# tsnb66/afivo-streamer

Measured on AMD Instinct MI355X. Metric: cell-updates/s (fluid+MG V-cycle), higher is better.
Workload: dtype f64; 1 GPU; s1-64; n_cell=64, leaf_cells=134217728, boxes=585, levels=4, coarse_solve=exact separable, fused_rhs=interior, face_field=from phi in the flux, vcycle_graphs=False, parallelism=single-gpu

## Files before the change

afivo-streamer_amd/csrc/afh_species.hip:

```cpp
#include <algorithm>
#include <type_traits>
#include <utility>

#include "afh_internal.h"
#include "afh_networks.h"

namespace afh {

constexpr int MAXS = AFH_MAX_SPECIES;
constexpr int MAXPREV = 4;

__device__ __forceinline__ size_t fidx(int nf, int d, int i, int j, int k) {
  return (size_t)d * nf * nf * nf + ((size_t)(k - 1) * nf + (j - 1)) * nf +
         (i - 1);
}

struct DevLT {
  int n_points, n_cols;
  double x_min, inv_fac;
  const double *rc;
  const double *rm = nullptr;
};

__device__ __forceinline__ double lt_col(const DevLT &lt, int col, double x) {
// ... 564 lines not shown
  const double *c = R.c;
  const double Tg = A.Tg;
  const double kB = 1.3806503e-23, eV = 1.6022e-19;
  const double electron_eV_to_K = 2 * eV / (3 * kB);
  if ((R.rate_type == AFH_RATE_K1 || R.rate_type == AFH_RATE_K3) && Te < 0)
    Te = electron_eV_to_K * lt_col(A.td, A.te_col, field);
  switch (R.rate_type) {
  case AFH_RATE_K1: return c0 * c[0] * pow(300 / Te, c[1]);
  case AFH_RATE_K3: {
    const double z = (kB / eV) * Te + c[1];
    return c0 * (c[0] * (z * z) - c[2]) * c[3];
  }
  case AFH_RATE_K4: return c0 * c[0] * pow(Tg / 300, c[1]) * exp(-c[2] / Tg);
  case AFH_RATE_K5: return c0 * c[0] * exp(-c[1] / Tg);
  case AFH_RATE_K6: return c0 * c[0] * pow(Tg, c[1]);
  case AFH_RATE_K7: return c0 * c[0] * pow(Tg / c[1], c[2]);
  case AFH_RATE_K8: return c0 * c[0] * pow(300 / Tg, c[1]);
  case AFH_RATE_K9: return c0 * c[0] * exp(-c[1] * Tg);
  case AFH_RATE_K10: return c0 * pow(10.0, c[0] + c[1] * (Tg - 300));
  case AFH_RATE_K11: return c0 * c[0] * pow(300 / Tg, c[1]) * exp(-c[2] / Tg);
  case AFH_RATE_K12: return c0 * c[0] * pow(Tg, c[1]) * exp(-c[2] / Tg);
  case AFH_RATE_K13: return c0 * c[0] * exp(-pow(c[1] / (c[2] + field), c[3]));
  case AFH_RATE_K14: return c0 * c[0] * exp(-pow(field / c[1], c[2]));
  default:
    return c0 * c[0] * exp(-pow(c[1] / (kB * (Tg + field / c[2])), c[3]));
  }
}

__device__ __forceinline__ double lt_at_rm(const DevLT &lt, int col, int low, double lf) {
  const double *r = lt.rm + (size_t)(low - 1) * lt.n_cols + (col - 1);
  return lf * r[0] + (1 - lf) * r[lt.n_cols];
}

template <bool SLOW>
__device__ __forceinline__ double rate_of(const UpdArgs &A, const DevReaction &R,
                                          double field, double &Te, int low = -1,
                                          double lf = 0.0) {
  const double c0 = R.rate_factor;
  const double *c = R.c;
  switch (R.rate_type) {
  case AFH_RATE_TABULATED_FIELD:
    return c0 * (low > 0 ? lt_at_rm(A.chem, R.table_col, low, lf)
                         : lt_col(A.chem, R.table_col, field));
  case AFH_RATE_CONSTANT: return c0 * c[0];
  case AFH_RATE_LINEAR: return c0 * c[0] * (field - c[1]);
  case AFH_RATE_EXP_V1: {
    const double z = c[1] / (c[2] + field);
    return c0 * c[0] * exp(-(z * z));
  }
  case AFH_RATE_EXP_V2: {
    const double z = field / c[1];
    return c0 * c[0] * exp(-(z * z));
  }
  default: return SLOW ? rate_slow(A, R, field, Te) : 0.0;
  }
}

template <int T, bool SLOW>
__device__ __forceinline__ double rate_t(const UpdArgs &A, const DevReaction &R, double field,
                                         double &Te, int low, double lf) {
  const double c0 = R.rate_factor;
  const double *c = R.c;
  if constexpr (T == AFH_RATE_TABULATED_FIELD) {
    return c0 * (low > 0 ? lt_at_rm(A.chem, R.table_col, low, lf)
                         : lt_col(A.chem, R.table_col, field));
  } else if constexpr (T == AFH_RATE_CONSTANT) {
    return c0 * c[0];
  } else if constexpr (T == AFH_RATE_LINEAR) {
    return c0 * c[0] * (field - c[1]);
  } else if constexpr (T == AFH_RATE_EXP_V1) {
    const double z = c[1] / (c[2] + field);
    return c0 * c[0] * exp(-(z * z));
  } else if constexpr (T == AFH_RATE_EXP_V2) {
    const double z = field / c[1];
    return c0 * c[0] * exp(-(z * z));
  } else {
    static_assert(SLOW, "temperature-dependent rate form in a fast update");
    return rate_slow(A, R, field, Te);
  }
}

template <class NET>
constexpr bool net_slow() {
  for (int r = 0; r < NET::NR; r++)
    if (NET::type[r] > AFH_RATE_EXP_V2) return true;
  return false;
}

template <class NET>
constexpr int net_slot(int ix) {
  return ix <= NET::NG ? NET::NS + ix - 1 : ix - NET::NG - 1;
}

template <class NET, bool SLOW, int R, int NT>
__device__ __forceinline__ void net_one(const UpdArgs &A, double field, double &Te, int clow,
                                        double clf, const double (&dens)[NT], double (&der)[NT]) {
  constexpr int NI = NET::n_in[R], NO = NET::n_out[R];
  const DevReaction &X = A.reac[R];
  double rate = rate_t<NET::type[R], SLOW>(A, X, field, Te, clow, clf);
  double prod = 1.0;
  if constexpr (NI > 0) prod = prod * dens[net_slot<NET>(NET::ix_in[R][0])];
  if constexpr (NI > 1) prod = prod * dens[net_slot<NET>(NET::ix_in[R][1])];
  if constexpr (NI > 2) prod = prod * dens[net_slot<NET>(NET::ix_in[R][2])];
  if constexpr (NI > 3) prod = prod * dens[net_slot<NET>(NET::ix_in[R][3])];
  rate = rate * prod;
  if constexpr (NI > 0) der[net_slot<NET>(NET::ix_in[R][0])] += -rate;
  if constexpr (NI > 1) der[net_slot<NET>(NET::ix_in[R][1])] += -rate;
  if constexpr (NI > 2) der[net_slot<NET>(NET::ix_in[R][2])] += -rate;
  if constexpr (NI > 3) der[net_slot<NET>(NET::ix_in[R][3])] += -rate;
  if constexpr (NO > 0) der[net_slot<NET>(NET::ix_out[R][0])] += rate * NET::mult[R][0];
  if constexpr (NO > 1) der[net_slot<NET>(NET::ix_out[R][1])] += rate * NET::mult[R][1];
  if constexpr (NO > 2) der[net_slot<NET>(NET::ix_out[R][2])] += rate * NET::mult[R][2];
  if constexpr (NO > 3) der[net_slot<NET>(NET::ix_out[R][3])] += rate * NET::mult[R][3];
}

template <class NET, bool SLOW, int NT, size_t... R>
__device__ __forceinline__ void net_all(const UpdArgs &A, double field, double &Te, int clow,
                                        double clf, const double (&dens)[NT], double (&der)[NT],
                                        std::index_sequence<R...>) {
  (net_one<NET, SLOW, (int)R, NT>(A, field, Te, clow, clf, dens, der), ...);
}

template <class NET>
struct net_nr {
  static constexpr int v = NET::NR;
};
template <>
struct net_nr<void> {
  static constexpr int v = 1;
};

template <class NET>
static bool net_matches(const afh_fluid_desc *d) {
  const bool gas = d->i_gas_dens > 0;
  if (d->n_species != NET::NS || d->n_reactions != NET::NR || gas != (NET::GAS != 0) ||
      (gas && d->n_gas_species != NET::NG))
    return false;
  for (int r = 0; r < NET::NR; r++) {
    const afh_reaction &a = d->reactions[r];
    if (a.rate_type != NET::type[r] || a.n_in != NET::n_in[r] || a.n_out != NET::n_out[r])
      return false;
    for (int q = 0; q < a.n_in; q++)
      if (a.ix_in[q] != NET::ix_in[r][q]) return false;
    for (int q = 0; q < a.n_out; q++)
      if (a.ix_out[q] != NET::ix_out[r][q] || a.mult_out[q] != NET::mult[r][q]) return false;
  }
  return true;
}

#ifndef AFH_FLUX_LDS_NT
// ... 538 lines not shown
#undef AFH_NET_CASE
  default: break;
  }
  if (A.Ng)
    hipLaunchKernelGGL((k_update<NS, true, MAXPREV, true, true>), grid, dim3(256), 0,
                       t->stream, A, ids, nc, t->bsz, t->fsz, red);
  else if (slow && A.n_prev == 1 && !sd)
    hipLaunchKernelGGL((k_update<NS, true, 1, false>), grid, dim3(256), 0, t->stream, A,
                       ids, nc, t->bsz, t->fsz, red);
  else if (slow && A.n_prev == 2 && !sd)
    hipLaunchKernelGGL((k_update<NS, true, 2, false>), grid, dim3(256), 0, t->stream, A,
                       ids, nc, t->bsz, t->fsz, red);
  else if (slow)
    hipLaunchKernelGGL((k_update<NS, true>), grid, dim3(256), 0, t->stream, A,
                       ids, nc, t->bsz, t->fsz, red);
  else if (A.n_prev == 1 && !sd)
    hipLaunchKernelGGL((k_update<NS, false, 1, false>), grid, dim3(256), 0,
                       t->stream, A, ids, nc, t->bsz, t->fsz, red);
  else if (A.n_prev == 2 && !sd)
    hipLaunchKernelGGL((k_update<NS, false, 2, false>), grid, dim3(256), 0,
                       t->stream, A, ids, nc, t->bsz, t->fsz, red);
  else
    hipLaunchKernelGGL((k_update<NS, false>), grid, dim3(256), 0, t->stream, A,
                       ids, nc, t->bsz, t->fsz, red);
}

#ifndef AFH_FE_NT
#define AFH_FE_NT 256
#endif
#ifndef AFH_FE_MINW
#define AFH_FE_MINW 3
#endif
constexpr int FE_CHEM_LDS = 2048;
template <int NC, int LIM, int NS, int NP, bool SD, bool PHI = false, class NET = void,
          bool WF = false, int NTT = AFH_FE_NT>
__global__ void __launch_bounds__(NTT, AFH_FE_MINW)
    k_fe_lds(FluxArgs A, UpdArgs U, const double *__restrict__ tdi,
             const int32_t *__restrict__ ids, size_t bsz, size_t fsz,
             unsigned long long *red) {
  constexpr bool wf = WF;
  using G = FluxLds<NC, NTT>;
  constexpr int NG = NC + 2, NF = NC + 1, TJ = G::TJ, NT = G::NT, RW = G::RW,
                NR = G::NR, EW = G::EW, ER = G::ER, NPE = G::NPE, EPE = G::EPE;
  constexpr int SK = NG * NG, FSK = NF * NF, FD = NF * NF * NF;
  constexpr int NN = NC * NC;
  constexpr bool HAS_NET = !std::is_void<NET>::value;
  extern __shared__ double T[];
  __shared__ double SN[2][NR * RW], SE[2][ER * EW];
  __shared__ double sv[NT], sd[NT], sf[NT];
  __shared__ double r1[NT / 64], r2[NT / 64], r3[NT / 64], r4[NT / 64];
  const int tid = threadIdx.x;
  const int wg = xcd_swizzle(blockIdx.x, gridDim.x);
  const int id = ids[wg / G::NTILE];
  const int i = tid % NC + 1;
  const int jr = tid / NC;
  const int j0 = (wg % G::NTILE) * TJ + 1, j = j0 + jr;
  const size_t boff = (size_t)(id - 1) * bsz;
  const double *ne = A.ne + boff;
  const double *E = A.E + boff;
  const double *Ef = A.Ef + (size_t)(id - 1) * fsz;
  const double *ph = PHI ? A.phi + boff : nullptr;
  double *F = A.F + (size_t)(id - 1) * fsz;
  const double *g2 = A.gc2 + (size_t)(id - 1) * 6 * NN;
  const double ix = A.inv_dx[0], iy = A.inv_dx[1], iz = A.inv_dx[2];
  const double gfx = A.gfac[0], gfy = A.gfac[1], gfz = A.gfac[2];
  const double N_inv = A.N_inv;
  const int np = A.td.n_points;
  const int eix = U.e_index, dq = U.der_q, ns = HAS_NET ? NS : U.ns;
  for (int e = tid; e < 2 * np; e += NT) T[e] = tdi[e];
  constexpr int NRS = net_nr<NET>::v;
  __shared__ DevReaction sreac[NRS];
  if (HAS_NET) {
    const int nw = (int)(sizeof(DevReaction) / sizeof(int)) * NRS;
    for (int e = tid; e < nw; e += NT)
      reinterpret_cast<int *>(sreac)[e] = reinterpret_cast<const int *>(U.reac)[e];
  }
  UpdArgs Ul = U;
  if (HAS_NET) Ul.reac = sreac;
  if constexpr (HAS_NET) {
    double *Tc = T + 2 * np;
    const int nch = U.chem.n_points * U.chem.n_cols;
    for (int e = tid; e < nch; e += NT) Tc[e] = U.chem.rm[e];
    Ul.chem.rm = Tc;
  }

  auto ne_at = [&](int k, int e) -> double {
    if (e >= NR * RW) return 0.0;
    const int jj = j0 - 2 + e / RW, ii = e % RW - 1;
    const bool jin = jj >= 0 && jj <= NC + 1, iin = ii >= 0 && ii <= NC + 1;
    if (jin && iin) return ne[(k * NG + jj) * NG + ii];
    if (jin && jj >= 1 && jj <= NC) {
      if (ii == -1) return g2[0 * NN + (k - 1) * NC + (jj - 1)];
      if (ii == NC + 2) return g2[1 * NN + (k - 1) * NC + (jj - 1)];
    }
    if (iin && ii >= 1 && ii <= NC) {
      if (jj == -1) return g2[2 * NN + (k - 1) * NC + (ii - 1)];
      if (jj == NC + 2) return g2[3 * NN + (k - 1) * NC + (ii - 1)];
    }
    return 0.0;
  };
  auto e_at = [&](int k, int e) -> double {
    if (e >= ER * EW) return 0.0;
    return E[(k * NG + (j0 - 1 + e / EW)) * NG + e % EW];
  };
  const int cc = j * NG + i;
  const int fcol = (j - 1) * NF + (i - 1);
  const int gz = (j - 1) * NC + (i - 1);
  double zm1 = ne[cc], z0 = ne[SK + cc], zp1 = ne[2 * SK + cc];
  const double zm2 = g2[4 * NN + gz];
#pragma unroll
  for (int q = 0; q < NPE; q++) {
    const int e = tid + NT * q;
    if (e < NR * RW) SN[1][e] = ne_at(1, e);
  }
#pragma unroll
  for (int q = 0; q < EPE; q++) {
    const int e = tid + NT * q;
    if (e < ER * EW) SE[1][e] = e_at(1, e);
  }
  double exl, eyl, exh, eyh, pk = 0.0;
  if (PHI) {
    const int c1 = SK + cc;
    pk = ph[c1];
    exl = gfx * (pk - ph[c1 - 1]);
    eyl = gfy * (pk - ph[c1 - NG]);
    exh = i == NC ? gfx * (ph[c1 + 1] - pk) : 0.0;
    eyh = (jr == TJ - 1) ? gfy * (ph[c1 + NG] - pk) : 0.0;
  } else {
    exl = Ef[fcol], eyl = Ef[FD + fcol];
    exh = i == NC ? Ef[fcol + 1] : 0.0;
    eyh = (jr == TJ - 1) ? Ef[FD + fcol + NF] : 0.0;
  }
  double mu, dcv;
  double cmax = -HUGE_VAL, smax = -HUGE_VAL, cmin = 1e100, rmax = 0.0;
  double vz_lo, dz_lo, fz_lo;
  {
    const double ezl = PHI ? gfz * (pk - ph[cc]) : Ef[2 * FD + fcol];
    const double u = upwind_t<LIM>(A.lim, zm2, zm1, z0, zp1, ezl);
    lds_mu_dc(tdi, A.td, 0.5 * (E[cc] + E[SK + cc]) * 1e21 * N_inv, mu, dcv);
    mu = mu * N_inv;
    dz_lo = dcv * N_inv;
    vz_lo = -mu * ezl;
    fz_lo = vz_lo * u - dz_lo * iz * (z0 - zm1);
    if (wf) F[2 * FD + fcol] = fz_lo;
    smax = fmax(smax, mu * u);
  }
  __syncthreads();

  const int cn = (jr + 2) * RW + (i + 1);
  const int ce = (jr + 1) * EW + i;

  for (int k = 1; k <= NC; k++) {
    const double *N0 = SN[k & 1], *E0p = SE[k & 1];
    const bool more = k < NC;
    const double zp2 = k + 2 <= NC + 1 ? ne[(k + 2) * SK + cc]
                                       : g2[5 * NN + gz];
    const double ep1 = E[(k + 1) * SK + cc];
    const int fbn = k * FSK + fcol;
    const int x = k * SK + cc;
    double ezh, nexl = 0, neyl = 0, nexh = 0, neyh = 0, npk = 0;
    if (PHI) {
      const int cn1 = (k + 1) * SK + cc;
      npk = ph[cn1];
      if (more) {
        nexl = ph[cn1 - 1];
        neyl = ph[cn1 - NG];
        if (i == NC) nexh = ph[cn1 + 1];
        if (jr == TJ - 1) neyh = ph[cn1 + NG];
      }
      ezh = gfz * (npk - pk);
    } else {
      ezh = Ef[2 * FD + fbn];
      if (more) {
        nexl = Ef[fbn];
        neyl = Ef[FD + fbn];
        if (i == NC) nexh = Ef[fbn + 1];
        if (jr == TJ - 1) neyh = Ef[FD + fbn + NF];
      }
    }
    double pv[NS][NP], dv[NS];
#pragma unroll
    for (int s = 0; s < NS; s++) {
#pragma unroll
      for (int q = 0; q < NP; q++)
        pv[s][q] = (s >= ns || (!SD && s == eix && q == dq)) ? 0.0
                                                              : (U.prev[s][q] + boff)[x];
      dv[s] = (!SD || s >= ns || s == eix) ? 0.0 : (U.der[s] + boff)[x];
    }
    double pn[NPE], pe[EPE];
#pragma unroll
    for (int q = 0; q < NPE; q++) pn[q] = more ? ne_at(k + 1, tid + NT * q) : 0.0;
#pragma unroll
    for (int q = 0; q < EPE; q++) pe[q] = more ? e_at(k + 1, tid + NT * q) : 0.0;

    const int fb = (k - 1) * FSK + fcol;
    const double e0 = E0p[ce];
    double vx, dx, fx;
    {
      const double u = upwind_t<LIM>(A.lim, N0[cn - 2], N0[cn - 1], z0, N0[cn + 1], exl);
      lds_mu_dc(T, A.td, 0.5 * (E0p[ce - 1] + e0) * 1e21 * N_inv, mu, dcv);
      mu = mu * N_inv;
      dx = dcv * N_inv;
      vx = -mu * exl;
      fx = vx * u - dx * ix * (z0 - N0[cn - 1]);
      if (wf) F[fb] = fx;
      smax = fmax(smax, mu * u);
    }
    double vxh = __shfl_down(vx, 1, 64), dxh = __shfl_down(dx, 1, 64);
    double fxh = __shfl_down(fx, 1, 64);
    if (i == NC) {
      const double u = upwind_t<LIM>(A.lim, N0[cn - 1], z0, N0[cn + 1], N0[cn + 2], exh);
      lds_mu_dc(T, A.td, 0.5 * (e0 + E0p[ce + 1]) * 1e21 * N_inv, mu, dcv);
      mu = mu * N_inv;
      dxh = dcv * N_inv;
      vxh = -mu * exh;
      fxh = vxh * u - dxh * ix * (N0[cn + 1] - z0);
      if (wf) F[fb + 1] = fxh;
      smax = fmax(smax, mu * u);
    }
    double vy, dy, fy;
    {
      const double u = upwind_t<LIM>(A.lim, N0[cn - 2 * RW], N0[cn - RW], z0,
                                     N0[cn + RW], eyl);
      lds_mu_dc(T, A.td, 0.5 * (E0p[ce - EW] + e0) * 1e21 * N_inv, mu, dcv);
      mu = mu * N_inv;
      dy = dcv * N_inv;
      vy = -mu * eyl;
      fy = vy * u - dy * iy * (z0 - N0[cn - RW]);
      if (wf) F[FD + fb] = fy;
      smax = fmax(smax, mu * u);
    }
    sv[tid] = vy;
    sd[tid] = dy;
    sf[tid] = fy;
    __syncthreads();
    double vyh, dyh, fyh;
    if (jr + 1 < TJ) {
      vyh = sv[tid + NC];
      dyh = sd[tid + NC];
      fyh = sf[tid + NC];
    } else {
      const double u = upwind_t<LIM>(A.lim, N0[cn - RW], z0, N0[cn + RW],
                                     N0[cn + 2 * RW], eyh);
      lds_mu_dc(T, A.td, 0.5 * (e0 + E0p[ce + EW]) * 1e21 * N_inv, mu, dcv);
      mu = mu * N_inv;
      dyh = dcv * N_inv;
      vyh = -mu * eyh;
      fyh = vyh * u - dyh * iy * (N0[cn + RW] - z0);
      if (j == NC) {
        if (wf) F[FD + fb + NF] = fyh;
        smax = fmax(smax, mu * u);
      }
    }
    double vzh, dzh, fzh;
    {
      const double u = upwind_t<LIM>(A.lim, zm1, z0, zp1, zp2, ezh);
      lds_mu_dc(T, A.td, 0.5 * (e0 + ep1) * 1e21 * N_inv, mu, dcv);
      mu = mu * N_inv;
      dzh = dcv * N_inv;
      vzh = -mu * ezh;
      fzh = vzh * u - dzh * iz * (zp1 - z0);
      if (wf) F[2 * FD + fb + FSK] = fzh;
      smax = fmax(smax, mu * u);
    }
    {
      const double mvx = fmax(fabs(vxh), fabs(vx)), mdx = fmax(dxh, dx);
      const double mvy = fmax(fabs(vyh), fabs(vy)), mdy = fmax(dyh, dy);
      double c = 0.0;
      c = c + (1.0 * mvx * ix + 2 * mdx * (ix * ix));
      c = c + (1.0 * mvy * iy + 2 * mdy * (iy * iy));
      const double mv = fmax(fabs(vzh), fabs(vz_lo));
      const double md = fmax(dzh, dz_lo);
      cmax = fmax(cmax, c + (1.0 * mv * iz + 2 * md * (iz * iz)));
    }
    {
      double y[NS], der[NS], dens[NS];
#pragma unroll
      for (int s = 0; s < NS; s++) {
#pragma unroll
        for (int q = 0; q < NP; q++)
          if (!SD && s == eix && q == dq) pv[s][q] = z0;
        if (SD && s == eix) dv[s] = z0;
        double tmp = 0.0;
#pragma unroll
        for (int q = 0; q < NP; q++) tmp = tmp + U.w_prev[q] * pv[s][q];
        y[s] = tmp;
        double v = dv[s];
#pragma unroll
        for (int q = 0; q < NP; q++)
          if (!SD && q == dq) v = pv[s][q];
        dens[s] = v > 0.0 ? v : 0.0;
        der[s] = 0.0;
      }
      const double field = 1e21 * U.inv_N * e0;
      double Te = -1.0;
      int clow = -1;
      double clf = 0.0;
      if (U.chem.rm) lt_loc(U.chem, field, clow, clf);
      if constexpr (HAS_NET) {
        net_all<NET, false>(Ul, field, Te, clow, clf, dens, der,
                            std::make_index_sequence<NET::NR>{});
      } else {
        for (int r = 0; r < U.nr; r++) {
          const DevReaction &R = U.reac[r];
          double rate = rate_of<false>(U, R, field, Te, clow, clf);
          double prod = 1.0;
          for (int q = 0; q < R.n_in; q++) prod = prod * sel(dens, R.ix_in[q] - 1);
          rate = rate * prod;
          for (int q = 0; q < R.n_in; q++) add_at(der, R.ix_in[q] - 1, -rate);
          for (int q = 0; q < R.n_out; q++)
            add_at(der, R.ix_out[q] - 1, rate * R.mult_out[q]);
        }
      }
      if (U.last_step) {
        const double eps = 1e-100;
#pragma unroll
        for (int s = 0; s < NS; s++) {
          if (s >= ns) break;
          double a, b;
          if (U.dt_chemistry_nmin > 0) {
            a = dens[s] + U.dt_chemistry_nmin;
            b = fabs(der[s]);
            b = b > eps ? b : eps;
          } else {
            a = dens[s] > eps ? dens[s] : eps;
            b = -der[s] > eps ? -der[s] : eps;
          }
          cmin = fmin(cmin, a / b);
        }
      }
#pragma unroll
      for (int s = 0; s < NS; s++) y[s] = y[s] + U.dt * der[s];
      const double div = U.dt_dr[0] * (fx - fxh);
      const double dvy = U.dt_dr[1] * (fy - fyh);
      const double dvz = U.dt_dr[2] * (fz_lo - fzh);
#pragma unroll
      for (int s = 0; s < NS; s++)
        if (s == eix) y[s] = y[s] + div + dvy + dvz;
#pragma unroll
      for (int s = 0; s < NS; s++)
        if (s < ns) st_nt<AFH_NT_UPD>(U.out[s] + boff + x, y[s]);
      if (U.rhs) {
        double r = 0.0;
#pragma unroll
        for (int s = 0; s < NS; s++)
          if (s < ns && U.rq[s] != 0.0) r = r + U.rq[s] * y[s];
        st_nt<AFH_NT_UPD>(U.rhs + boff + x, r);
        rmax = fmax(rmax, fabs(r));
      }
    }
    if (more) {
#pragma unroll
      for (int q = 0; q < NPE; q++) {
        const int e = tid + NT * q;
        if (e < NR * RW) SN[(k + 1) & 1][e] = pn[q];
      }
#pragma unroll
      for (int q = 0; q < EPE; q++) {
        const int e = tid + NT * q;
        if (e < ER * EW) SE[(k + 1) & 1][e] = pe[q];
      }
    }
    zm1 = z0;
    z0 = zp1;
    zp1 = zp2;
    vz_lo = vzh, dz_lo = dzh, fz_lo = fzh;
    if (PHI) {
      if (more) {
        exl = gfx * (npk - nexl);
        eyl = gfy * (npk - neyl);
        exh = i == NC ? gfx * (nexh - npk) : 0.0;
        eyh = (jr == TJ - 1) ? gfy * (neyh - npk) : 0.0;
      }
      pk = npk;
    } else {
      exl = nexl, eyl = neyl, exh = nexh, eyh = neyh;
    }
    __syncthreads();
  }
  for (int o = 32; o > 0; o >>= 1) {
    cmax = fmax(cmax, __shfl_xor(cmax, o, 64));
    smax = fmax(smax, __shfl_xor(smax, o, 64));
    cmin = fmin(cmin, __shfl_xor(cmin, o, 64));
    rmax = fmax(rmax, __shfl_xor(rmax, o, 64));
  }
  const int lane = tid & 63, w = tid >> 6;
  if (lane == 0) r1[w] = cmax, r2[w] = smax, r3[w] = cmin, r4[w] = rmax;
  __syncthreads();
// ... 874 lines not shown
  int slots[2], n_fold = 0;
  bool mx[2];
  if (A.rhs) slots[n_fold] = 4, mx[n_fold++] = true;
  if (last_step) slots[n_fold] = 2, mx[n_fold++] = false;
  return n_fold ? red_finish_n(t, n_fold, slots, mx) : AFH_OK;
}

extern "C" {

int32_t afh_flux_update_densities(afh_fluid *f, double dt, int32_t s_deriv,
                                  int32_t n_prev, const int32_t *s_prev,
                                  const double *w_prev, int32_t s_out,
                                  int32_t last_step, double *dt_lim) {
  if (!f || !dt_lim) return set_error(AFH_ERR_ARG, "afh_flux_update_densities: null");
  afh_tree *t = f->t;
  AFH_LIVE(t, "afh_flux_update_densities");
  int32_t e;
  if ((e = update_dev(f, dt, s_deriv, n_prev, s_prev, w_prev, s_out, last_step))) return e;
  double r = 1e100;
  if (last_step) {
    if ((e = red_reduce_fetch(t, 2, 0, 1, &r))) return e;
  } else {
    AFH_HIP(hipStreamSynchronize(t->stream));
  }
  dt_lim[0] = r;
  dt_lim[1] = 1e100;
  return AFH_OK;
}

}

constexpr int FE_MAX_SPECIES = 4;

template <int NC, int NS, int NP, bool SD, bool PHI, class NET>
static void launch_fe(afh_tree *t, const FluxArgs &A, const UpdArgs &U,
                      const double *tdi, int l, unsigned long long *red, int wf) {
  using G = FluxLds<NC, AFH_FE_NT>;
  const dim3 grid(t->leaves.n(l) * G::NTILE);
  size_t lds = 2 * sizeof(double) * A.td.n_points;
  if (!std::is_void<NET>::value) lds += sizeof(double) * U.chem.n_points * U.chem.n_cols;
  if (wf)
    hipLaunchKernelGGL((k_fe_lds<NC, AFH_LIM_KOREN, NS, NP, SD, PHI, NET, true>), grid,
                       dim3(G::NT), lds, t->stream, A, U, tdi, t->leaves.at(l), t->bsz,
                       t->fsz, red);
  else
    hipLaunchKernelGGL((k_fe_lds<NC, AFH_LIM_KOREN, NS, NP, SD, PHI, NET, false>), grid,
                       dim3(G::NT), lds, t->stream, A, U, tdi, t->leaves.at(l), t->bsz,
                       t->fsz, red);
}

template <int NC>
static void launch_fe_nc(afh_tree *t, const FluxArgs &A, const UpdArgs &U,
                         const double *tdi, int l, unsigned long long *red, int wf,
                         int net) {
  const bool sd = U.der_q < 0, phi = A.phi != nullptr;
  const int v = (U.n_prev == 2 ? 1 : 0) | (sd ? 2 : 0) | (phi ? 4 : 0);
#define AFH_FE_CASES(NSX, NETX)                                                    \
  switch (v) {                                                                     \
  case 0: launch_fe<NC, NSX, 1, false, false, NETX>(t, A, U, tdi, l, red, wf); break; \
  case 1: launch_fe<NC, NSX, 2, false, false, NETX>(t, A, U, tdi, l, red, wf); break; \
  case 2: launch_fe<NC, NSX, 1, true, false, NETX>(t, A, U, tdi, l, red, wf); break;  \
  case 3: launch_fe<NC, NSX, 2, true, false, NETX>(t, A, U, tdi, l, red, wf); break;  \
  case 4: launch_fe<NC, NSX, 1, false, true, NETX>(t, A, U, tdi, l, red, wf); break;  \
  case 5: launch_fe<NC, NSX, 2, false, true, NETX>(t, A, U, tdi, l, red, wf); break;  \
  case 6: launch_fe<NC, NSX, 1, true, true, NETX>(t, A, U, tdi, l, red, wf); break;   \
  default: launch_fe<NC, NSX, 2, true, true, NETX>(t, A, U, tdi, l, red, wf); break;  \
  }
  if (net == 1) {
    AFH_FE_CASES(net::Airsiglo::NS, net::Airsiglo)
  } else {
    AFH_FE_CASES(FE_MAX_SPECIES, void)
  }
#undef AFH_FE_CASES
}

extern "C" {

}

static int32_t fetch_step(afh_fluid *f, int32_t last_step, int n_extra, const int32_t *extra,
                          double *dt_lim, double *extra_out) {
  int32_t slots[RED_SLOTS];
  double r[RED_SLOTS];
  int n = 0;
  slots[n++] = AFH_SLOT_CFL;
  slots[n++] = AFH_SLOT_SIGMA;
  if (last_step) slots[n++] = AFH_SLOT_CHEM;
  if (n_extra < 0 || n_extra > 2)
    return set_error(AFH_ERR_ARG, "afh_fluid_fetch_step: %d extra slots", n_extra);
  for (int q = 0; q < n_extra; q++) {
    if (extra[q] != AFH_SLOT_MAXRES && extra[q] != AFH_SLOT_RHS)
      return set_error(AFH_ERR_ARG, "afh_fluid_fetch_step: slot %d", extra[q]);
    slots[n++] = extra[q];
  }
  int32_t e;
  if ((e = red_fetch_slots(f->t, n, slots, r))) return e;
  flux_dt_limits(r, dt_lim);
  dt_lim[2] = last_step ? r[2] : 1e100;
  dt_lim[3] = 1e100;
  for (int q = 0; q < n_extra; q++) extra_out[q] = r[n - n_extra + q];
  return AFH_OK;
}

static int32_t fe_dev(afh_fluid *f, double dt, int32_t s_deriv, int32_t n_prev,
                      const int32_t *s_prev, const double *w_prev, int32_t s_out,
                      int32_t last_step, int32_t store_flux) {
  afh_tree *t = f->t;
  const int nc = t->nc, n3 = nc * nc * nc;
  const int iv = f->d.i_electron + s_deriv;
  if (iv < 1 || iv > t->nvc) return set_error(AFH_ERR_ARG, "bad s_deriv");
  UpdArgs U;
  double upd_bytes;
  int32_t e;
  if ((e = upd_args(f, dt, s_deriv, n_prev, s_prev, w_prev, s_out, last_step, U,
                    upd_bytes)))
    return e;
  bool alias = false;
  for (int s = 0; s < f->d.n_species; s++) {
    const int ivo = f->d.species_iv[s] + s_out;
    alias |= ivo == iv || ivo == f->d.i_efld;
  }
  const char *fused_env = getenv("AFH_FE_FUSED");
  const int fe_mode = fused_env ? atoi(fused_env) : 1;
  const bool net_ok =
      (f->net == 1 && f->chem.rm && f->chem.n_points * f->chem.n_cols <= FE_CHEM_LDS) ||
      (f->net == 0 && f->d.n_species <= FE_MAX_SPECIES);
  const bool policy = fe_mode == 2 || (fe_mode == 1 && nc == 64);
  const bool fused = policy && f->d_tdi &&
                     (nc == 16 || nc == 32 || nc == 64) && !t->any_cflux &&
                     !f->slow_rates && net_ok && f->d.i_gas_dens <= 0 &&
                     f->d.i_photo <= 0 && n_prev <= 2 && !alias &&
                     f->d.limiter == AFH_LIM_KOREN && f->d.n_ions == 0 && !f->mask_iv;
  if (!fused) {
    if ((e = flux_tree_dev(f, s_deriv))) return e;
    if (f->d.n_ions > 0 && f->ion_se_yield > 0 && (e = ion_se_dev(f))) return e;
    return update_dev(f, dt, s_deriv, n_prev, s_prev, w_prev, s_out, last_step);
  }
  t->touch(iv);
  f->rhs_state = -1;
  if ((e = flux_prelude(f, iv, t->gc2))) return e;
  if ((e = red_init(t, 0, -HUGE_VAL)) || (e = red_init(t, 1, -HUGE_VAL)) ||
      (e = red_init(t, 2, 1e100)) || (U.rhs && (e = red_init(t, 4, 0.0))))
    return e;
  auto *red = reinterpret_cast<unsigned long long *>(t->scratch);
  const FluxArgs A0 = flux_args(f, iv);
  const double fe_bytes =
      upd_bytes - (f->phi_iv > 0 ? 16.0 : 0.0) + (store_flux ? 24.0 : 0.0);
  for (int l = 1; l <= t->nlvl; l++) {
    const int n = t->leaves.n(l);
    if (!n) continue;
    FluxArgs A = A0;
    for (int q = 0; q < 3; q++) {
      A.inv_dx[q] = 1 / t->lvl_dr[3 * (l - 1) + q];
      A.gfac[q] = A.fac / t->lvl_dr[3 * (l - 1) + q];
      U.dt_dr[q] = dt / t->lvl_dr[3 * (l - 1) + q];
    }
    prof_begin(t, AFH_PROF_FE);
    switch (nc) {
// ... 171 lines not shown
```

Measured before the change: 12.70 billion cell-updates/s.

## Slim fused flux-update kernel args, specialize der_q/e_index, precompute halo offsets

Result: faster. 12.99 billion cell-updates/s, median of 6 (+2.3%).

```diff
diff --git a/afivo-streamer_amd/csrc/afh_species.hip b/afivo-streamer_amd/csrc/afh_species.hip
--- a/afivo-streamer_amd/csrc/afh_species.hip
+++ b/afivo-streamer_amd/csrc/afh_species.hip
@@ -620,8 +620,8 @@
   return lf * r[0] + (1 - lf) * r[lt.n_cols];
 }
 
-template <bool SLOW>
-__device__ __forceinline__ double rate_of(const UpdArgs &A, const DevReaction &R,
+template <bool SLOW, class ARGS>
+__device__ __forceinline__ double rate_of(const ARGS &A, const DevReaction &R,
                                           double field, double &Te, int low = -1,
                                           double lf = 0.0) {
   const double c0 = R.rate_factor;
@@ -640,12 +640,14 @@
     const double z = field / c[1];
     return c0 * c[0] * exp(-(z * z));
   }
-  default: return SLOW ? rate_slow(A, R, field, Te) : 0.0;
-  }
-}
-
-template <int T, bool SLOW>
-__device__ __forceinline__ double rate_t(const UpdArgs &A, const DevReaction &R, double field,
+  default:
+    if constexpr (SLOW) return rate_slow(A, R, field, Te);
+    return 0.0;
+  }
+}
+
+template <int T, bool SLOW, class ARGS>
+__device__ __forceinline__ double rate_t(const ARGS &A, const DevReaction &R, double field,
                                          double &Te, int low, double lf) {
   const double c0 = R.rate_factor;
   const double *c = R.c;
@@ -680,8 +682,8 @@
   return ix <= NET::NG ? NET::NS + ix - 1 : ix - NET::NG - 1;
 }
 
-template <class NET, bool SLOW, int R, int NT>
-__device__ __forceinline__ void net_one(const UpdArgs &A, double field, double &Te, int clow,
+template <class NET, bool SLOW, int R, int NT, class ARGS>
+__device__ __forceinline__ void net_one(const ARGS &A, double field, double &Te, int clow,
                                         double clf, const double (&dens)[NT], double (&der)[NT]) {
   constexpr int NI = NET::n_in[R], NO = NET::n_out[R];
   const DevReaction &X = A.reac[R];
@@ -702,8 +704,8 @@
   if constexpr (NO > 3) der[net_slot<NET>(NET::ix_out[R][3])] += rate * NET::mult[R][3];
 }
 
-template <class NET, bool SLOW, int NT, size_t... R>
-__device__ __forceinline__ void net_all(const UpdArgs &A, double field, double &Te, int clow,
+template <class NET, bool SLOW, class ARGS, int NT, size_t... R>
+__device__ __forceinline__ void net_all(const ARGS &A, double field, double &Te, int clow,
                                         double clf, const double (&dens)[NT], double (&der)[NT],
                                         std::index_sequence<R...>) {
   (net_one<NET, SLOW, (int)R, NT>(A, field, Te, clow, clf, dens, der), ...);
@@ -1308,17 +1310,90 @@
 #define AFH_FE_MINW 3
 #endif
 constexpr int FE_CHEM_LDS = 2048;
-template <int NC, int LIM, int NS, int NP, bool SD, bool PHI = false, class NET = void,
-          bool WF = false, int NTT = AFH_FE_NT>
+
+template <int NS, int NP, int ND>
+struct FeArgs {
+  const double *ne;
+  const double *E;
+  const double *fld;
+  const double *gc2;
+  double *F;
+  const double *prev[NS][NP];
+  const double *der[ND > 0 ? ND : 1];
+  double *out[NS];
+  double *rhs;
+  unsigned long long *rhs_red;
+  const DevReaction *reac;
+  DevLT td, chem;
+  double N_inv;
+  double inv_dx[3], gfac[3], dt_dr[3];
+  double inv_dx2[3];
+  double e21_inv_N;
+  double td_last, chem_last;
+  double dt, dt_chemistry_nmin;
+  double w_prev[NP], rq[NS];
+  int lim, ns, nr, last_step, e_index;
+};
+
+struct FeChem {
+  const DevReaction *reac;
+  DevLT chem;
+};
+
+__device__ __forceinline__ void fe_lt_loc(const DevLT &lt, double last, double x, int &low,
+                                          double &lf) {
+  const double frac = (x - lt.x_min) * lt.inv_fac;
+  const bool lo = frac <= 0, hi = frac >= last;
+  const int c = (int)ceil(frac);
+  low = lo ? 1 : hi ? lt.n_points - 1 : c;
+  lf = lo ? 1.0 : hi ? 0.0 : c - frac;
+}
+
+__device__ __forceinline__ void fe_mu_dc(const double *T, const DevLT &lt, double last,
+                                         double x, double &mu, double &dc) {
+  int low;
+  double lf;
+  fe_lt_loc(lt, last, x, low, lf);
+  const double *r = T + 2 * (low - 1);
+  mu = lf * r[0] + (1 - lf) * r[2];
+  dc = lf * r[1] + (1 - lf) * r[3];
+}
+
+template <class T>
+__device__ __forceinline__ T *fe_at(T *base, unsigned b) {
+  using B = std::conditional_t<std::is_const<T>::value, const char, char>;
+  return reinterpret_cast<T *>(reinterpret_cast<B *>(base) + b);
+}
+
+template <int LIM>
+__device__ __forceinline__ double fe_upwind(int lim, double Lm2, double Lm1, double L0,
+                                            double Lp1, double ex) {
+  if (LIM == AFH_LIM_KOREN) {
+    const bool up = -1 * ex > 0;
+    const double a = L0 - Lm1, b = up ? Lm1 - Lm2 : Lp1 - L0;
+    const double aa = a * a, ab = a * b;
+    double l = 2 * b;
+    l = aa <= 2.5 * ab ? (1 / 3.0) * (b + 2 * a) : l;
+    l = aa <= 0.25 * ab ? 2 * a : l;
+    l = ab <= 0 ? 0.0 : l;
+    return up ? Lm1 + 0.5 * l : L0 - 0.5 * l;
+  }
+  return upwind_t<LIM>(lim, Lm2, Lm1, L0, Lp1, ex);
+}
+
+template <int NC, int LIM, int NS, int NP, int DQ, bool PHI = false, class NET = void,
+          bool WF = false, int EIX = -1, int NTT = AFH_FE_NT>
 __global__ void __launch_bounds__(NTT, AFH_FE_MINW)
-    k_fe_lds(FluxArgs A, UpdArgs U, const double *__restrict__ tdi,
+    k_fe_lds(FeArgs<NS, NP, (DQ < 0 ? NS : 0)> U, const double *__restrict__ tdi,
              const int32_t *__restrict__ ids, size_t bsz, size_t fsz,
              unsigned long long *red) {
   constexpr bool wf = WF;
+  constexpr bool SD = DQ < 0;
   using G = FluxLds<NC, NTT>;
   constexpr int NG = NC + 2, NF = NC + 1, TJ = G::TJ, NT = G::NT, RW = G::RW,
                 NR = G::NR, EW = G::EW, ER = G::ER, NPE = G::NPE, EPE = G::EPE;
   constexpr int SK = NG * NG, FSK = NF * NF, FD = NF * NF * NF;
+  constexpr unsigned SKB = SK * 8, FSKB = FSK * 8, FDB = FD * 8;
   constexpr int NN = NC * NC;
   constexpr bool HAS_NET = !std::is_void<NET>::value;
   extern __shared__ double T[];
@@ -1332,17 +1407,23 @@
   const int jr = tid / NC;
   const int j0 = (wg % G::NTILE) * TJ + 1, j = j0 + jr;
   const size_t boff = (size_t)(id - 1) * bsz;
-  const double *ne = A.ne + boff;
-  const double *E = A.E + boff;
-  const double *Ef = A.Ef + (size_t)(id - 1) * fsz;
-  const double *ph = PHI ? A.phi + boff : nullptr;
-  double *F = A.F + (size_t)(id - 1) * fsz;
-  const double *g2 = A.gc2 + (size_t)(id - 1) * 6 * NN;
-  const double ix = A.inv_dx[0], iy = A.inv_dx[1], iz = A.inv_dx[2];
-  const double gfx = A.gfac[0], gfy = A.gfac[1], gfz = A.gfac[2];
-  const double N_inv = A.N_inv;
-  const int np = A.td.n_points;
-  const int eix = U.e_index, dq = U.der_q, ns = HAS_NET ? NS : U.ns;
+  const double *ne = U.ne + boff;
+  const double *E = U.E + boff;
+  const double *Ef = PHI ? nullptr : U.fld + (size_t)(id - 1) * fsz;
+  const double *ph = PHI ? U.fld + boff : nullptr;
+  double *F = wf ? U.F + (size_t)(id - 1) * fsz : nullptr;
+  const double *g2 = U.gc2 + (size_t)(id - 1) * 6 * NN;
+  const double ix = U.inv_dx[0], iy = U.inv_dx[1], iz = U.inv_dx[2];
+  const double ix2 = U.inv_dx2[0], iy2 = U.inv_dx2[1], iz2 = U.inv_dx2[2];
+  const double gfx = U.gfac[0], gfy = U.gfac[1], gfz = U.gfac[2];
+  const double dtx = U.dt_dr[0], dty = U.dt_dr[1], dtz = U.dt_dr[2];
+  const double N_inv = U.N_inv;
+  const DevLT td = U.td;
+  const double td_last = U.td_last;
+  const int lim = U.lim;
+  const int np = td.n_points;
+  const int eix = EIX >= 0 ? EIX : U.e_index, ns = HAS_NET ? NS : U.ns;
+  constexpr int dq = DQ;
   for (int e = tid; e < 2 * np; e += NT) T[e] = tdi[e];
   constexpr int NRS = net_nr<NET>::v;
   __shared__ DevReaction sreac[NRS];
@@ -1351,8 +1432,7 @@
     for (int e = tid; e < nw; e += NT)
       reinterpret_cast<int *>(sreac)[e] = reinterpret_cast<const int *>(U.reac)[e];
   }
-  UpdArgs Ul = U;
-  if (HAS_NET) Ul.reac = sreac;
+  FeChem Ul{HAS_NET ? sreac : U.reac, U.chem};
   if constexpr (HAS_NET) {
     double *Tc = T + 2 * np;
     const int nch = U.chem.n_points * U.chem.n_cols;
@@ -1360,39 +1440,43 @@
     Ul.chem.rm = Tc;
   }
 
-  auto ne_at = [&](int k, int e) -> double {
-    if (e >= NR * RW) return 0.0;
+  int sn[NPE], so[EPE];
+#pragma unroll
+  for (int q = 0; q < NPE; q++) {
+    const int e = tid + NT * q < NR * RW ? tid + NT * q : 0;
     const int jj = j0 - 2 + e / RW, ii = e % RW - 1;
     const bool jin = jj >= 0 && jj <= NC + 1, iin = ii >= 0 && ii <= NC + 1;
-    if (jin && iin) return ne[(k * NG + jj) * NG + ii];
-    if (jin && jj >= 1 && jj <= NC) {
-      if (ii == -1) return g2[0 * NN + (k - 1) * NC + (jj - 1)];
-      if (ii == NC + 2) return g2[1 * NN + (k - 1) * NC + (jj - 1)];
-    }
-    if (iin && ii >= 1 && ii <= NC) {
-      if (jj == -1) return g2[2 * NN + (k - 1) * NC + (ii - 1)];
-      if (jj == NC + 2) return g2[3 * NN + (k - 1) * NC + (ii - 1)];
-    }
-    return 0.0;
+    const bool gx = jj >= 1 && jj <= NC && (ii == -1 || ii == NC + 2);
+    const bool gy = ii >= 1 && ii <= NC && (jj == -1 || jj == NC + 2);
+    const int go = gx ? (ii == -1 ? 0 : NN) + (jj - 1) : (jj == -1 ? 2 * NN : 3 * NN) + (ii - 1);
+    sn[q] = jin && iin ? (jj * NG + ii) * 8 : (gx || gy) ? ~(go * 8) : (int)SKB;
+  }
+  auto ne_at = [&](int q, int kk) -> double {
+    const int o = sn[q];
+    return o >= 0 ? *fe_at(ne, kk * SKB + o) : *fe_at(g2, (kk - 1) * (NC * 8) + ~o);
   };
-  auto e_at = [&](int k, int e) -> double {
-    if (e >= ER * EW) return 0.0;
-    return E[(k * NG + (j0 - 1 + e / EW)) * NG + e % EW];
-  };
+#pragma unroll
+  for (int q = 0; q < EPE; q++) {
+    const int e = tid + NT * q < ER * EW ? tid + NT * q : 0;
+    so[q] = ((j0 - 1 + e / EW) * NG + e % EW) * 8;
+  }
   const int cc = j * NG + i;
   const int fcol = (j - 1) * NF + (i - 1);
   const int gz = (j - 1) * NC + (i - 1);
+  const unsigned ccb = cc * 8, fcb = fcol * 8;
   double zm1 = ne[cc], z0 = ne[SK + cc], zp1 = ne[2 * SK + cc];
   const double zm2 = g2[4 * NN + gz];
 #pragma unroll
   for (int q = 0; q < NPE; q++) {
     const int e = tid + NT * q;
-    if (e < NR * RW) SN[1][e] = ne_at(1, e);
+    const double v = ne_at(q, 1);
+    if (e < NR * RW) SN[1][e] = sn[q] == (int)SKB ? 0.0 : v;
   }
 #pragma unroll
   for (int q = 0; q < EPE; q++) {
     const int e = tid + NT * q;
-    if (e < ER * EW) SE[1][e] = e_at(1, e);
+    const double v = *fe_at(E, SKB + so[q]);
+    if (e < ER * EW) SE[1][e] = v;
   }
   double exl, eyl, exh, eyh, pk = 0.0;
   if (PHI) {
@@ -1412,8 +1496,8 @@
   double vz_lo, dz_lo, fz_lo;
   {
     const double ezl = PHI ? gfz * (pk - ph[cc]) : Ef[2 * FD + fcol];
-    const double u = upwind_t<LIM>(A.lim, zm2, zm1, z0, zp1, ezl);
-    lds_mu_dc(tdi, A.td, 0.5 * (E[cc] + E[SK + cc]) * 1e21 * N_inv, mu, dcv);
+    const double u = fe_upwind<LIM>(lim, zm2, zm1, z0, zp1, ezl);
+    fe_mu_dc(tdi, td, td_last, 0.5 * (E[cc] + E[SK + cc]) * 1e21 * N_inv, mu, dcv);
     mu = mu * N_inv;
     dz_lo = dcv * N_inv;
     vz_lo = -mu * ezl;
@@ -1429,29 +1513,28 @@
   for (int k = 1; k <= NC; k++) {
     const double *N0 = SN[k & 1], *E0p = SE[k & 1];
     const bool more = k < NC;
-    const double zp2 = k + 2 <= NC + 1 ? ne[(k + 2) * SK + cc]
-                                       : g2[5 * NN + gz];
-    const double ep1 = E[(k + 1) * SK + cc];
-    const int fbn = k * FSK + fcol;
-    const int x = k * SK + cc;
+    const unsigned xb = k * SKB + ccb;
+    const unsigned fbn = k * FSKB + fcb;
+    const double zp2 = k + 2 <= NC + 1 ? *fe_at(ne, xb + 2 * SKB) : g2[5 * NN + gz];
+    const double ep1 = *fe_at(E, xb + SKB);
     double ezh, nexl = 0, neyl = 0, nexh = 0, neyh = 0, npk = 0;
     if (PHI) {
-      const int cn1 = (k + 1) * SK + cc;
-      npk = ph[cn1];
+      const unsigned cn1 = xb + SKB;
+      npk = *fe_at(ph, cn1);
       if (more) {
-        nexl = ph[cn1 - 1];
-        neyl = ph[cn1 - NG];
-        if (i == NC) nexh = ph[cn1 + 1];
-        if (jr == TJ - 1) neyh = ph[cn1 + NG];
+        nexl = *fe_at(ph, cn1 - 8);
+        neyl = *fe_at(ph, cn1 - NG * 8);
+        if (i == NC) nexh = *fe_at(ph, cn1 + 8);
+        if (jr == TJ - 1) neyh = *fe_at(ph, cn1 + NG * 8);
       }
       ezh = gfz * (npk - pk);
     } else {
-      ezh = Ef[2 * FD + fbn];
+      ezh = *fe_at(Ef, 2 * FDB + fbn);
       if (more) {
-        nexl = Ef[fbn];
-        neyl = Ef[FD + fbn];
-        if (i == NC) nexh = Ef[fbn + 1];
-        if (jr == TJ - 1) neyh = Ef[FD + fbn + NF];
+        nexl = *fe_at(Ef, fbn);
+        neyl = *fe_at(Ef, FDB + fbn);
+        if (i == NC) nexh = *fe_at(Ef, fbn + 8);
+        if (jr == TJ - 1) neyh = *fe_at(Ef, FDB + fbn + NF * 8);
       }
     }
     double pv[NS][NP], dv[NS];
@@ -1460,50 +1543,56 @@
 #pragma unroll
       for (int q = 0; q < NP; q++)
         pv[s][q] = (s >= ns || (!SD && s == eix && q == dq)) ? 0.0
-                                                              : (U.prev[s][q] + boff)[x];
-      dv[s] = (!SD || s >= ns || s == eix) ? 0.0 : (U.der[s] + boff)[x];
+                                                              : *fe_at(U.prev[s][q] + boff, xb);
+      dv[s] = (!SD || s >= ns || s == eix) ? 0.0 : *fe_at(U.der[SD ? s : 0] + boff, xb);
     }
     double pn[NPE], pe[EPE];
 #pragma unroll
-    for (int q = 0; q < NPE; q++) pn[q] = more ? ne_at(k + 1, tid + NT * q) : 0.0;
-#pragma unroll
-    for (int q = 0; q < EPE; q++) pe[q] = more ? e_at(k + 1, tid + NT * q) : 0.0;
-
-    const int fb = (k - 1) * FSK + fcol;
+    for (int q = 0; q < NPE; q++) pn[q] = 0.0;
+#pragma unroll
+    for (int q = 0; q < EPE; q++) pe[q] = 0.0;
+    if (more) {
+#pragma unroll
+      for (int q = 0; q < NPE; q++) pn[q] = ne_at(q, k + 1);
+#pragma unroll
+      for (int q = 0; q < EPE; q++) pe[q] = *fe_at(E, (k + 1) * SKB + so[q]);
+    }
+
+    const unsigned fb = fbn - FSKB;
     const double e0 = E0p[ce];
     double vx, dx, fx;
     {
-      const double u = upwind_t<LIM>(A.lim, N0[cn - 2], N0[cn - 1], z0, N0[cn + 1], exl);
-      lds_mu_dc(T, A.td, 0.5 * (E0p[ce - 1] + e0) * 1e21 * N_inv, mu, dcv);
+      const double u = fe_upwind<LIM>(lim, N0[cn - 2], N0[cn - 1], z0, N0[cn + 1], exl);
+      fe_mu_dc(T, td, td_last, 0.5 * (E0p[ce - 1] + e0) * 1e21 * N_inv, mu, dcv);
       mu = mu * N_inv;
       dx = dcv * N_inv;
       vx = -mu * exl;
       fx = vx * u - dx * ix * (z0 - N0[cn - 1]);
-      if (wf) F[fb] = fx;
+      if (wf) *fe_at(F, fb) = fx;
       smax = fmax(smax, mu * u);
     }
     double vxh = __shfl_down(vx, 1, 64), dxh = __shfl_down(dx, 1, 64);
     double fxh = __shfl_down(fx, 1, 64);
     if (i == NC) {
-      const double u = upwind_t<LIM>(A.lim, N0[cn - 1], z0, N0[cn + 1], N0[cn + 2], exh);
-      lds_mu_dc(T, A.td, 0.5 * (e0 + E0p[ce + 1]) * 1e21 * N_inv, mu, dcv);
+      const double u = fe_upwind<LIM>(lim, N0[cn - 1], z0, N0[cn + 1], N0[cn + 2], exh);
+      fe_mu_dc(T, td, td_last, 0.5 * (e0 + E0p[ce + 1]) * 1e21 * N_inv, mu, dcv);
       mu = mu * N_inv;
       dxh = dcv * N_inv;
       vxh = -mu * exh;
       fxh = vxh * u - dxh * ix * (N0[cn + 1] - z0);
-      if (wf) F[fb + 1] = fxh;
+      if (wf) *fe_at(F, fb + 8) = fxh;
       smax = fmax(smax, mu * u);
     }
     double vy, dy, fy;
     {
-      const double u = upwind_t<LIM>(A.lim, N0[cn - 2 * RW], N0[cn - RW], z0,
+      const double u = fe_upwind<LIM>(lim, N0[cn - 2 * RW], N0[cn - RW], z0,
                                      N0[cn + RW], eyl);
-      lds_mu_dc(T, A.td, 0.5 * (E0p[ce - EW] + e0) * 1e21 * N_inv, mu, dcv);
+      fe_mu_dc(T, td, td_last, 0.5 * (E0p[ce - EW] + e0) * 1e21 * N_inv, mu, dcv);
       mu = mu * N_inv;
       dy = dcv * N_inv;
       vy = -mu * eyl;
       fy = vy * u - dy * iy * (z0 - N0[cn - RW]);
-      if (wf) F[FD + fb] = fy;
+      if (wf) *fe_at(F, FDB + fb) = fy;
       smax = fmax(smax, mu * u);
     }
     sv[tid] = vy;
@@ -1516,38 +1605,38 @@
       dyh = sd[tid + NC];
       fyh = sf[tid + NC];
     } else {
-      const double u = upwind_t<LIM>(A.lim, N0[cn - RW], z0, N0[cn + RW],
+      const double u = fe_upwind<LIM>(lim, N0[cn - RW], z0, N0[cn + RW],
                                      N0[cn + 2 * RW], eyh);
-      lds_mu_dc(T, A.td, 0.5 * (e0 + E0p[ce + EW]) * 1e21 * N_inv, mu, dcv);
+      fe_mu_dc(T, td, td_last, 0.5 * (e0 + E0p[ce + EW]) * 1e21 * N_inv, mu, dcv);
       mu = mu * N_inv;
       dyh = dcv * N_inv;
       vyh = -mu * eyh;
       fyh = vyh * u - dyh * iy * (N0[cn + RW] - z0);
       if (j == NC) {
-        if (wf) F[FD + fb + NF] = fyh;
+        if (wf) *fe_at(F, FDB + fb + NF * 8) = fyh;
         smax = fmax(smax, mu * u);
       }
     }
     double vzh, dzh, fzh;
     {
-      const double u = upwind_t<LIM>(A.lim, zm1, z0, zp1, zp2, ezh);
-      lds_mu_dc(T, A.td, 0.5 * (e0 + ep1) * 1e21 * N_inv, mu, dcv);
+      const double u = fe_upwind<LIM>(lim, zm1, z0, zp1, zp2, ezh);
+      fe_mu_dc(T, td, td_last, 0.5 * (e0 + ep1) * 1e21 * N_inv, mu, dcv);
       mu = mu * N_inv;
       dzh = dcv * N_inv;
       vzh = -mu * ezh;
       fzh = vzh * u - dzh * iz * (zp1 - z0);
-      if (wf) F[2 * FD + fb + FSK] = fzh;
+      if (wf) *fe_at(F, 2 * FDB + fbn) = fzh;
       smax = fmax(smax, mu * u);
     }
     {
       const double mvx = fmax(fabs(vxh), fabs(vx)), mdx = fmax(dxh, dx);
       const double mvy = fmax(fabs(vyh), fabs(vy)), mdy = fmax(dyh, dy);
       double c = 0.0;
-      c = c + (1.0 * mvx * ix + 2 * mdx * (ix * ix));
-      c = c + (1.0 * mvy * iy + 2 * mdy * (iy * iy));
+      c = c + (1.0 * mvx * ix + 2 * mdx * ix2);
+      c = c + (1.0 * mvy * iy + 2 * mdy * iy2);
       const double mv = fmax(fabs(vzh), fabs(vz_lo));
       const double md = fmax(dzh, dz_lo);
-      cmax = fmax(cmax, c + (1.0 * mv * iz + 2 * md * (iz * iz)));
+      cmax = fmax(cmax, c + (1.0 * mv * iz + 2 * md * iz2));
     }
     {
       double y[NS], der[NS], dens[NS];
@@ -1568,18 +1657,18 @@
         dens[s] = v > 0.0 ? v : 0.0;
         der[s] = 0.0;
       }
-      const double field = 1e21 * U.inv_N * e0;
+      const double field = U.e21_inv_N * e0;
       double Te = -1.0;
       int clow = -1;
       double clf = 0.0;
-      if (U.chem.rm) lt_loc(U.chem, field, clow, clf);
+      if (U.chem.rm) fe_lt_loc(U.chem, U.chem_last, field, clow, clf);
       if constexpr (HAS_NET) {
         net_all<NET, false>(Ul, field, Te, clow, clf, dens, der,
                             std::make_index_sequence<NET::NR>{});
       } else {
         for (int r = 0; r < U.nr; r++) {
           const DevReaction &R = U.reac[r];
-          double rate = rate_of<false>(U, R, field, Te, clow, clf);
+          double rate = rate_of<false>(Ul, R, field, Te, clow, clf);
           double prod = 1.0;
           for (int q = 0; q < R.n_in; q++) prod = prod * sel(dens, R.ix_in[q] - 1);
           rate = rate * prod;
@@ -1607,21 +1696,21 @@
       }
 #pragma unroll
       for (int s = 0; s < NS; s++) y[s] = y[s] + U.dt * der[s];
-      const double div = U.dt_dr[0] * (fx - fxh);
-      const double dvy = U.dt_dr[1] * (fy - fyh);
-      const double dvz = U.dt_dr[2] * (fz_lo - fzh);
+      const double div = dtx * (fx - fxh);
+      const double dvy = dty * (fy - fyh);
+      const double dvz = dtz * (fz_lo - fzh);
 #pragma unroll
       for (int s = 0; s < NS; s++)
         if (s == eix) y[s] = y[s] + div + dvy + dvz;
 #pragma unroll
       for (int s = 0; s < NS; s++)
-        if (s < ns) st_nt<AFH_NT_UPD>(U.out[s] + boff + x, y[s]);
+        if (s < ns) st_nt<AFH_NT_UPD>(fe_at(U.out[s] + boff, xb), y[s]);
       if (U.rhs) {
         double r = 0.0;
 #pragma unroll
         for (int s = 0; s < NS; s++)
           if (s < ns && U.rq[s] != 0.0) r = r + U.rq[s] * y[s];
-        st_nt<AFH_NT_UPD>(U.rhs + boff + x, r);
+        st_nt<AFH_NT_UPD>(fe_at(U.rhs + boff, xb), r);
         rmax = fmax(rmax, fabs(r));
       }
     }
@@ -1629,7 +1718,7 @@
 #pragma unroll
       for (int q = 0; q < NPE; q++) {
         const int e = tid + NT * q;
-        if (e < NR * RW) SN[(k + 1) & 1][e] = pn[q];
+        if (e < NR * RW) SN[(k + 1) & 1][e] = sn[q] == (int)SKB ? 0.0 : pn[q];
       }
 #pragma unroll
       for (int q = 0; q < EPE; q++) {
@@ -2570,39 +2659,77 @@
 
 constexpr int FE_MAX_SPECIES = 4;
 
-template <int NC, int NS, int NP, bool SD, bool PHI, class NET>
+constexpr int FE_NET_EIX = 0;
+
+template <int NC, int NS, int NP, int DQ, bool PHI, class NET>
 static void launch_fe(afh_tree *t, const FluxArgs &A, const UpdArgs &U,
                       const double *tdi, int l, unsigned long long *red, int wf) {
   using G = FluxLds<NC, AFH_FE_NT>;
+  constexpr int EIX = std::is_void<NET>::value ? -1 : FE_NET_EIX;
   const dim3 grid(t->leaves.n(l) * G::NTILE);
   size_t lds = 2 * sizeof(double) * A.td.n_points;
   if (!std::is_void<NET>::value) lds += sizeof(double) * U.chem.n_points * U.chem.n_cols;
+  FeArgs<NS, NP, (DQ < 0 ? NS : 0)> X{};
+  X.ne = A.ne;
+  X.E = A.E;
+  X.fld = PHI ? A.phi : A.Ef;
+  X.gc2 = A.gc2;
+  X.F = wf ? A.F : nullptr;
+  for (int s = 0; s < NS; s++) {
+    const bool in = s < U.ns;
+    for (int q = 0; q < NP; q++) X.prev[s][q] = in ? U.prev[s][q] : nullptr;
+    if constexpr (DQ < 0) X.der[s] = in ? U.der[s] : nullptr;
+    X.out[s] = in ? U.out[s] : nullptr;
+    X.rq[s] = in ? U.rq[s] : 0.0;
+  }
+  X.rhs = U.rhs;
+  X.rhs_red = U.rhs_red;
+  X.reac = U.reac;
+  X.td = A.td;
+  X.chem = U.chem;
+  X.N_inv = A.N_inv;
+  X.e21_inv_N = 1e21 * U.inv_N;
+  X.td_last = A.td.n_points - 1;
+  X.chem_last = U.chem.n_points - 1;
+  for (int q = 0; q < 3; q++)
+    X.inv_dx[q] = A.inv_dx[q], X.gfac[q] = A.gfac[q], X.dt_dr[q] = U.dt_dr[q],
+    X.inv_dx2[q] = A.inv_dx[q] * A.inv_dx[q];
+  X.dt = U.dt;
+  X.dt_chemistry_nmin = U.dt_chemistry_nmin;
+  for (int q = 0; q < NP; q++) X.w_prev[q] = U.w_prev[q];
+  X.lim = A.lim;
+  X.ns = U.ns;
+  X.nr = U.nr;
+  X.last_step = U.last_step;
+  X.e_index = U.e_index;
   if (wf)
-    hipLaunchKernelGGL((k_fe_lds<NC, AFH_LIM_KOREN, NS, NP, SD, PHI, NET, true>), grid,
-                       dim3(G::NT), lds, t->stream, A, U, tdi, t->leaves.at(l), t->bsz,
-                       t->fsz, red);
+    hipLaunchKernelGGL((k_fe_lds<NC, AFH_LIM_KOREN, NS, NP, DQ, PHI, NET, true, EIX>), grid,
+                       dim3(G::NT), lds, t->stream, X, tdi, t->leaves.at(l), t->bsz, t->fsz,
+                       red);
   else
-    hipLaunchKernelGGL((k_fe_lds<NC, AFH_LIM_KOREN, NS, NP, SD, PHI, NET, false>), grid,
-                       dim3(G::NT), lds, t->stream, A, U, tdi, t->leaves.at(l), t->bsz,
-                       t->fsz, red);
+    hipLaunchKernelGGL((k_fe_lds<NC, AFH_LIM_KOREN, NS, NP, DQ, PHI, NET, false, EIX>), grid,
+                       dim3(G::NT), lds, t->stream, X, tdi, t->leaves.at(l), t->bsz, t->fsz,
+                       red);
 }
 
 template <int NC>
 static void launch_fe_nc(afh_tree *t, const FluxArgs &A, const UpdArgs &U,
                          const double *tdi, int l, unsigned long long *red, int wf,
                          int net) {
-  const bool sd = U.der_q < 0, phi = A.phi != nullptr;
-  const int v = (U.n_prev == 2 ? 1 : 0) | (sd ? 2 : 0) | (phi ? 4 : 0);
-#define AFH_FE_CASES(NSX, NETX)                                                    \
-  switch (v) {                                                                     \
-  case 0: launch_fe<NC, NSX, 1, false, false, NETX>(t, A, U, tdi, l, red, wf); break; \
-  case 1: launch_fe<NC, NSX, 2, false, false, NETX>(t, A, U, tdi, l, red, wf); break; \
-  case 2: launch_fe<NC, NSX, 1, true, false, NETX>(t, A, U, tdi, l, red, wf); break;  \
-  case 3: launch_fe<NC, NSX, 2, true, false, NETX>(t, A, U, tdi, l, red, wf); break;  \
-  case 4: launch_fe<NC, NSX, 1, false, true, NETX>(t, A, U, tdi, l, red, wf); break;  \
-  case 5: launch_fe<NC, NSX, 2, false, true, NETX>(t, A, U, tdi, l, red, wf); break;  \
-  case 6: launch_fe<NC, NSX, 1, true, true, NETX>(t, A, U, tdi, l, red, wf); break;   \
-  default: launch_fe<NC, NSX, 2, true, true, NETX>(t, A, U, tdi, l, red, wf); break;  \
+  const bool phi = A.phi != nullptr;
+  const int v = (U.n_prev == 2 ? 3 : 1) + U.der_q + (phi ? 5 : 0);
+#define AFH_FE_CASES(NSX, NETX)                                                     \
+  switch (v) {                                                                      \
+  case 0: launch_fe<NC, NSX, 1, -1, false, NETX>(t, A, U, tdi, l, red, wf); break;  \
+  case 1: launch_fe<NC, NSX, 1, 0, false, NETX>(t, A, U, tdi, l, red, wf); break;   \
+  case 2: launch_fe<NC, NSX, 2, -1, false, NETX>(t, A, U, tdi, l, red, wf); break;  \
+  case 3: launch_fe<NC, NSX, 2, 0, false, NETX>(t, A, U, tdi, l, red, wf); break;   \
+  case 4: launch_fe<NC, NSX, 2, 1, false, NETX>(t, A, U, tdi, l, red, wf); break;   \
+  case 5: launch_fe<NC, NSX, 1, -1, true, NETX>(t, A, U, tdi, l, red, wf); break;   \
+  case 6: launch_fe<NC, NSX, 1, 0, true, NETX>(t, A, U, tdi, l, red, wf); break;    \
+  case 7: launch_fe<NC, NSX, 2, -1, true, NETX>(t, A, U, tdi, l, red, wf); break;   \
+  case 8: launch_fe<NC, NSX, 2, 0, true, NETX>(t, A, U, tdi, l, red, wf); break;    \
+  default: launch_fe<NC, NSX, 2, 1, true, NETX>(t, A, U, tdi, l, red, wf); break;   \
   }
   if (net == 1) {
     AFH_FE_CASES(net::Airsiglo::NS, net::Airsiglo)
@@ -2661,7 +2788,8 @@
   const char *fused_env = getenv("AFH_FE_FUSED");
   const int fe_mode = fused_env ? atoi(fused_env) : 1;
   const bool net_ok =
-      (f->net == 1 && f->chem.rm && f->chem.n_points * f->chem.n_cols <= FE_CHEM_LDS) ||
+      (f->net == 1 && f->chem.rm && f->chem.n_points * f->chem.n_cols <= FE_CHEM_LDS &&
+       f->e_index == FE_NET_EIX) ||
       (f->net == 0 && f->d.n_species <= FE_MAX_SPECIES);
   const bool policy = fe_mode == 2 || (fe_mode == 1 && nc == 64);
   const bool fused = policy && f->d_tdi &&
```
